# comfy-creator/Comfy-Gen-Server

Measured on AMD Instinct MI355X. Metric: images/sec (whole node) + sec/image, SDXL 1024 20-step Euler-a at 1/2/4/8 MI355X, higher is better.
Workload: dtype bf16; 1 GPU; model=sdxl-base, global_batch=8, seq_len=16384, resolution=1024, sampler_steps=20, sampler=euler_ancestral, unet_batch_per_gpu=16, parallelism=dp1, pipelined=True

## Files before the change

### build_native.py

```python
#!/usr/bin/env python3
from __future__ import annotations

import concurrent.futures as cf
import glob
import json
import os
import subprocess
import sys
import sysconfig

ROOT = os.path.dirname(os.path.abspath(__file__))
PKG = os.path.join(ROOT, "comfy_gen_server_amd")
KDIR = os.path.join(PKG, "csrc", "kernels")
RDIR = os.path.join(PKG, "csrc", "runtime")
LIB = os.path.join(PKG, "lib")
BUILD = os.path.join(ROOT, "build", "native")
ROCM = os.environ.get("ROCM_PATH", "/opt/rocm")
HIPCC = os.path.join(ROCM, "bin", "hipcc")
ARCH = os.environ.get("CGS_OFFLOAD_ARCH", "gfx950")


def _run(cmd):
    r = subprocess.run(cmd, stdout=subprocess.PIPE, stderr=subprocess.STDOUT, text=True)
    if r.returncode != 0:
        raise RuntimeError("command failed:\n" + " ".join(cmd) + "\n" + r.stdout)
    return r.stdout


def _stale(src, obj, deps=()):
    if not os.path.exists(obj):
        return True
    t = os.path.getmtime(obj)
    return any(os.path.getmtime(p) > t for p in (src,) + tuple(deps))


SCRATCH_BUDGET = {"gemm_bf16_nt_v7_kernel": 128, "conv_nhwc_v7_kernel": 128, "attn_fwd_d64": 64}


def _resources(out):
    res, cur = {}, None
    for line in out.splitlines():
        if "remark:" not in line:
            continue
        txt = line.split("remark:", 1)[1].split("[-Rpass", 1)[0].strip()
        key, _, val = txt.partition(":")
        val = val.strip()
        if key == "Function Name":
            cur = val
            res[cur] = {}
        elif cur is not None and key in ("VGPRs", "AGPRs", "ScratchSize [bytes/lane]", "VGPRs Spill"):
            res[cur][{"VGPRs": "vgpr", "AGPRs": "agpr", "ScratchSize [bytes/lane]": "scratch",
                      "VGPRs Spill": "spill"}[key]] = int(val.split()[0])
    return res


def _check_resources(report):
    if not report:
        return
    path = os.path.join(BUILD, "kernel_resources.json")
    old = {}
    if os.path.exists(path):
        with open(path) as f:
            old = json.load(f)
    old.update(report)
    with open(path, "w") as f:
        json.dump(old, f, indent=1, sort_keys=True)
    bad = [(k, v.get("scratch", 0), lim) for k, v in report.items() for pat, lim in SCRATCH_BUDGET.items()
           if pat in k and v.get("scratch", 0) > lim]
    if bad:
# ... 92 lines not shown
```

### comfy_gen_server_amd/_native.py

```python
from __future__ import annotations

import ctypes
import glob
import os
import threading

_HERE = os.path.dirname(os.path.abspath(__file__))
LIB_DIR = os.path.join(_HERE, "lib")
_lock = threading.Lock()
_kernels = None
_kernels_err = None


def kernel_lib_path() -> str:
    return os.environ.get("CGS_KERNELS_SO") or os.path.join(LIB_DIR, "libcgs_kernels.so")


def load_kernels():
    global _kernels, _kernels_err
    if _kernels is not None or _kernels_err is not None:
        return _kernels
    with _lock:
        if _kernels is not None or _kernels_err is not None:
            return _kernels
# ... 54 lines not shown
    "cgs_euler_step": [_P, _P, _P, _L, _F, _F, _F, _P],
    "cgs_timestep_embedding": [_P, _P, _I, _I, _F, _I, _P],
    "cgs_silu": [_P, _P, _L, _I, _P],
    "cgs_act": [_P, _P, _L, _I, _F, _I, _P],
    "cgs_upsample_nearest2x_nhwc": [_P, _P, _I, _I, _I, _I, _I, _P],
    "cgs_dwconv_nhwc": [_P, _P, _P, _P, _I, _I, _I, _I, _I, _I, _I, _P],
    "cgs_dwconv_ln_stats_nhwc": [_P, _P, _P, _P, _P, _I, _I, _I, _I, _I, _I, _F, _I, _P],
    "cgs_conv2d_nhwc": [_P, _P, _P, _P, _P, _I, _I, _I, _I, _I, _I, _I, _I, _I, _I, _I, _P],
    "cgs_fused_bias_act": [_P, _P, _P, _L, _I, _L, _F, _F, _I, _P],
    "cgs_upfirdn2d": [_P, _P, _P, _I, _I, _I, _I, _I, _I, _I, _I, _I, _I, _I, _I, _I, _I, _P],
    "cgs_resize": [_P, _P, _I, _I, _I, _I, _I, _I, _I, _I, _P],
    "cgs_lanczos_u8_h": [_P, _L, _L, _L, _L, _P, _I, _I, _I, _I, _I, _P, _P, _I, _I, _I, _P],
    "cgs_lanczos_u8_v": [_P, _I, _L, _L, _L, _L, _P, _I, _I, _I, _I, _P, _P, _I, _P],
    "cgs_bislerp": [_P, _P, _I, _I, _I, _I, _L, _L, _L, _L, _I, _I, _P, _P, _P, _I, _I, _P],
    "cgs_vq_nearest": [_P, _P, _P, _P, _I, _I, _I, _I, _P],
    "cgs_grn_nhwc": [_P, _P, _P, _P, _P, _I, _I, _I, _I, _P],
    "cgs_grn_stats": [_P, _P, _I, _I, _I, _I, _I, _P],
    "cgs_splitk_ws_bytes": [_I, _I, _I],
    "cgs_gemm_bf16_splitk": [_P, _P, _P, _P, _P, _P, _P, _I, _I, _I, _L, _L, _L, _L, _I, _F, _I, _I, _P, _L, _P],
    "cgs_grn_stats_gns": [_P, _P, _I, _I, _I, _P],
    "cgs_grn_apply_gns": [_P, _P, _P, _P, _P, _P, _I, _I, _I, _P],
    "cgs_gemm_bf16_gelu_gns": [_P, _P, _P, _P, _P, _P, _I, _I, _I, _L, _L, _L, _I, _P, _I, _P],
    "cgs_grn_scale_weight": [_P, _P, _P, _I, _I, _I, _I, _P, _P],
    "cgs_h2d_upload": [_P, _P, _L, _L, _I, _P],
    "cgs_gemm_f32": [_P, _P, _P, _P, _P, _I, _I, _I, _L, _L, _L, _L, _I, _F, _I, _I, _L, _L, _L, _P],
    "cgs_conv_f32": [_P, _P, _P, _P, _P, _P, _I, _I, _I, _I, _I, _I, _I, _I, _I, _I, _I, _I, _I, _P],
    "cgs_groupnorm_f32_ws": [_I, _I, _I],
    "cgs_groupnorm_f32": [_P, _P, _I, _P, _P, _P, _P, _P, _I, _I, _I, _I, _F, _I, _P],
    "cgs_layernorm_f32": [_P, _P, _P, _P, _L, _I, _F, _P],
    "cgs_softmax_rows": [_P, _P, _L, _I, _F, _I, _P],
    "cgs_gemm_bf16_w8": [_P, _P, _P, _P, _P, _I, _I, _I, _L, _L, _L, _L, _I, _F, _P],
    "cgs_gemm_bf16_v": [_P, _P, _P, _P, _P, _I, _I, _I, _L, _L, _L, _L, _I, _F, _I, _P],
    "cgs_conv2d_nhwc_v": [_P, _P, _I, _P, _P, _P, _P, _I, _I, _I, _I, _I, _I, _I, _I, _I, _I, _I, _I, _I, _P],
    "cgs_upconv_taps_nhwc": [_P, _P, _P, _P, _I, _I, _I, _I, _I, _P],
    "cgs_conv2d_nhwc_act": [_P, _P, _I, _P, _P, _P, _P, _I, _I, _I, _I, _I, _I, _I, _I, _I, _I, _I, _I, _I, _I, _F,
                            _P],
    "cgs_philox_randn": [_P, _I, _L, ctypes.c_ulonglong, _L, ctypes.c_ulonglong, _P, _F, _I, _P, _P],
    "cgs_euler_ancestral_philox": [_P, _P, _I, _L, _F, _F, _F, ctypes.c_ulonglong, _L, ctypes.c_ulonglong, _P, _P],
    "cgs_brownian_increment": [_P, _I, _L, ctypes.c_ulonglong, _L, ctypes.c_double, ctypes.c_double,
                               ctypes.c_double, ctypes.c_double, ctypes.c_double, _I, _F, _P, _P],
    "cgs_sampler_step_dev": [_P, _P, _P, _P, _I, _L, _F, _P, _I, _P, _P],
    "cgs_step_param": [_P, _I, _P, _I, _I, _P, _P],
    "cgs_step_advance": [_P, _P],
    "cgs_vae_out_u8": [_P, _P, _L, _P],
    "cgs_conv2d_nhwc_ex": [_P, _P, _I, _P, _P, _P, _P, _I, _I, _I, _I, _I, _I, _I, _I, _I, _I, _I, _I, _P],
    "cgs_region_accumulate": [_P, _P, _P, _I, _P, _I, _I, _I, _I, _I, _I, _I, _I, _I, _L, _L, _L, _L, _I, _L, _L,
                              _L, _L, _I, _F, _P],
    "cgs_region_normalize": [_P, _P, _P, _L, _I, _P],
    "cgs_clip_embed": [_P, _P, _P, _P, _I, _I, _I, _I, _I, _P],
    "cgs_pooled_gather": [_P, _P, _P, _I, _I, _I, _I, _P],
    "cgs_layernorm_stats": [_P, _P, _I, _I, _F, _I, _P],
    "cgs_gemm_bf16_lnfold": [_P, _P, _P, _P, _P, _P, _I, _I, _I, _L, _L, _L, _I, _P, _L, _P],
    "cgs_gemm_bf16_lnfold_v": [_P, _P, _P, _P, _P, _P, _I, _I, _I, _L, _L, _L, _I, _P, _L, _I, _P],
    "cgs_v7_ws_bytes": [_I, _I, _I],
    "cgs_v7_set_dbg": [_I],
    "cgs_v6_set_mode": [_I],
    "cgs_attn_set_prio": [_I],
    "cgs_gn_set_blocks": [_I],
    "cgs_conv_smalln_set_lds": [_I],
    "cgs_attn_set_kv2_rows": [_I],
    "cgs_grn_set_rows": [_I],
    "cgs_flash_attn_fwd_ks": [_P, _P, _P, _P, _I, _I, _I, _I, _L, _L, _L, _L, _L, _L, _L, _L, _F, _I, _P, _P, _P],
    "cgs_flash_attn_fwd_kv2": [_P, _P, _P, _P, _P, _P, _I, _I, _I, _I, _I, _L, _L, _L, _L, _L, _L, _L, _L, _L, _L, _L, _L, _F, _P],
    "cgs_conv2d_nhwc_gns": [_P, _P, _I, _P, _P, _P, _P, _I, _I, _I, _I, _I, _I, _I, _I, _I, _I, _I, _I, _P, _P],
    "cgs_groupnorm_band_stats": [_P, _P, _I, _P, _P, _P, _I, _I, _I, _I, _I, _P],
    "cgs_groupnorm_apply_stats": [_P, _P, _I, _P, _P, _P, _P, _P, _P, _I, _I, _I, _I, _I, _I, _P],
# ... 75 lines not shown
```

### comfy_gen_server_amd/csrc/kernels/conv.hip

```cpp
#include "common.h"
#include <stdlib.h>
#include "mfma_core.h"
#include "mfma_pp.h"
#include "mfma_pp160.h"
#include "mfma_ppk.h"

#define EPI_BIAS 1
#define EPI_RESIDUAL 2
#define CONV_UP2X 16
#ifndef CGS_CONV_PFE
#define CGS_CONV_PFE 0
#endif

typedef __attribute__((address_space(3))) void lds_void;

__device__ __attribute__((aligned(16))) unsigned char g_conv_zero_page[256];

struct ConvArgs {
  const u16* in;
  const u16* in2;
  const u16* w;
  const u16* bias;
  const u16* res;
  u16* out;
  int N, H, W, Cin, C1, Cout, kh, kw, stride, pad, Ho, Wo;
  int flags;
  int tiles_n;
  int group_m;
  unsigned cq_magic;
  int kw_m16;
  ppk::Split sp;
  float* gnp;
  int img_rsrc;
  int act;
  float act_param;
};

__device__ __forceinline__ mc::Epi conv_epi(const ConvArgs& a) {
  return mc::Epi{a.out, a.bias, a.res, a.Cout, a.Cout, a.flags & (EPI_BIAS | EPI_RESIDUAL), 1.0f};
}
__device__ __forceinline__ mc::Epi conv_tile_epi(const ConvArgs& a) {
  mc::Epi e = conv_epi(a);
  if (a.act) {
    e.flags |= MC_EPI_GELU;
    e.act = a.act;
    e.act_param = a.act_param;
  }
  return e;
}

static void conv_magic(ConvArgs& a) {
  const unsigned cq = (unsigned)(a.Cin / 64);
  a.cq_magic = cq <= 1 ? 0u : (unsigned)(((1ull << 32) + cq - 1) / cq);
  a.kw_m16 = (65536 + a.kw - 1) / a.kw;
}

static long long conv_tiles(ConvArgs& a, int BM, int BN) {
  const int M = a.N * a.Ho * a.Wo;
  a.tiles_n = (a.Cout + BN - 1) / BN;
  return (long long)((M + BM - 1) / BM) * a.tiles_n;
}

template <auto Kern>
static void conv_run(const ConvArgs& a, long long grid, int threads, int lds, hipStream_t stream) {
  max_dynamic_lds_once<Kern>(lds);
  Kern<<<(unsigned)grid, threads, lds, stream>>>(a);
}

// ... 311 lines not shown
    const bool ok = row < M;
    row = ok ? row : M - 1;
    const int hw = a->Ho * a->Wo;
    const int n = row / hw;
    const int rem = row - n * hw;
    const int oy = rem / a->Wo;
    const int py = oy * a->stride - a->pad, px = (rem - oy * a->Wo) * a->stride - a->pad;
    pix[s] = (n * a->H + py) * a->W + px;
    uint32_t m = 0;
    if (ok) {
      for (int ky = 0; ky < a->kh; ++ky) {
        const bool ry = (unsigned)(py + ky) < (unsigned)a->H;
        for (int kx = 0; kx < a->kw; ++kx)
          if (ry && (unsigned)(px + kx) < (unsigned)a->W) m |= 1u << (ky * a->kw + kx);
      }
    }
    vm[s] = m;
  }
  __device__ __forceinline__ void dma(int s, int k0, unsigned char* dst) const {
    const unsigned kq = (unsigned)k0 >> 6;
    const unsigned tap = a->cq_magic ? __umulhi(kq, a->cq_magic) : kq;
    const int ci0 = k0 - (int)tap * a->Cin;
    const int ky = (int)((tap * (unsigned)a->kw_m16) >> 16);
    const int kx = (int)tap - ky * a->kw;
    const bool second = ci0 >= a->C1;
    const int cs = second ? a->Cin - a->C1 : a->C1;
    const int cb = (second ? ci0 - a->C1 : ci0) + 8 * pp::src_chunk8(s & 1);
    const unsigned p = (unsigned)(pix[s] + ky * a->W + kx);
    const unsigned off = ((vm[s] >> tap) & 1u) ? 2u * (p * (unsigned)cs + (unsigned)cb) : 0x80000000u;
    __builtin_amdgcn_raw_ptr_buffer_load_lds(second ? r2 : r1, (lds_void*)dst, 16, off, 0, 0, 0);
  }
};

struct ConvGatherKD {
  static constexpr bool kOwnDMA = true;
  const ConvArgs* a;
  uint32_t pb1[4], pb2[4], vm[4];
  __amdgpu_buffer_rsrc_t r1, r2;
  __device__ __forceinline__ void make(long long n_img, unsigned px) {
    const unsigned c2 = (unsigned)(a->in2 ? a->Cin - a->C1 : a->C1);
    r1 = __builtin_amdgcn_make_buffer_rsrc((void*)(a->in + n_img * px * a->C1), 0, (int)(px * (unsigned)a->C1 * 2u),
                                           0x00020000);
    r2 = __builtin_amdgcn_make_buffer_rsrc((void*)((a->in2 ? a->in2 : a->in) + n_img * px * c2), 0,
                                           (int)(px * c2 * 2u), 0x00020000);
  }
  __device__ __forceinline__ void init() {
    if (!a->img_rsrc) make(0, (unsigned)(a->N * a->H * a->W));
  }
  __device__ __forceinline__ void tile(int m0) {
    if (a->img_rsrc) make(m0 / (a->Ho * a->Wo), (unsigned)(a->H * a->W));
  }
  __device__ __forceinline__ void setup(int s, int row) {
    const int M = a->N * a->Ho * a->Wo;
    const bool ok = row < M;
    row = ok ? row : M - 1;
    const int hw = a->Ho * a->Wo;
    const int n = row / hw;
    const int rem = row - n * hw;
    const int oy = rem / a->Wo;
    const int py = oy * a->stride - a->pad, px = (rem - oy * a->Wo) * a->stride - a->pad;
    const unsigned pix = (unsigned)(((a->img_rsrc ? 0 : n) * a->H + py) * a->W + px);
    uint32_t m = 0;
    if (ok) {
      for (int ky = 0; ky < a->kh; ++ky) {
        const bool ry = (unsigned)(py + ky) < (unsigned)a->H;
        for (int kx = 0; kx < a->kw; ++kx)
          if (ry && (unsigned)(px + kx) < (unsigned)a->W) m |= 1u << (ky * a->kw + kx);
      }
    }
    vm[s] = m;
    const unsigned ch = 16u * (unsigned)pp::src_chunk8(s & 1);
    pb1[s] = pix * (2u * (unsigned)a->C1) + ch;
    pb2[s] = pix * (2u * (unsigned)(a->Cin - a->C1)) + ch;
  }
  __device__ __forceinline__ void dma(int s, int k0, unsigned char* dst) const {
    const unsigned kq = (unsigned)k0 >> 6;
    const unsigned tap = __umulhi(kq, a->cq_magic) + (a->cq_magic ? 0u : kq);
    const int ci0 = k0 - (int)tap * a->Cin;
    const int ky = (int)((tap * (unsigned)a->kw_m16) >> 16);
    const int kx = (int)tap - ky * a->kw;
    const bool second = ci0 >= a->C1;
    const unsigned cs2 = 2u * (unsigned)(second ? a->Cin - a->C1 : a->C1);
    const unsigned so = (unsigned)(ky * a->W + kx) * cs2 + 2u * (unsigned)(second ? ci0 - a->C1 : ci0);
    const unsigned off = ((second ? pb2[s] : pb1[s]) + so) | (~(vm[s] << (31u - tap)) & 0x80000000u);
    __builtin_amdgcn_raw_ptr_buffer_load_lds(second ? r2 : r1, (lds_void*)dst, 16, off, 0, 0, 0);
  }
};

struct ConvGatherKU {
  static constexpr bool kOwnDMA = true;
  const ConvArgs* a;
  uint32_t pb[4], vm[4];
  int py[4], px[4];
  __amdgpu_buffer_rsrc_t r1;
  __device__ __forceinline__ void make(long long n_img, unsigned pixels) {
    r1 = __builtin_amdgcn_make_buffer_rsrc((void*)(a->in + n_img * pixels * a->C1), 0,
                                           (int)(pixels * (unsigned)a->C1 * 2u), 0x00020000);
  }
  __device__ __forceinline__ void init() {
    if (!a->img_rsrc) make(0, (unsigned)(a->N * a->H * a->W));
  }
  __device__ __forceinline__ void tile(int m0) {
    if (a->img_rsrc) make(m0 / (a->Ho * a->Wo), (unsigned)(a->H * a->W));
  }
  __device__ __forceinline__ void setup(int s, int row) {
    const int M = a->N * a->Ho * a->Wo;
    const bool ok = row < M;
    row = ok ? row : M - 1;
    const int hw = a->Ho * a->Wo;
    const int n = row / hw;
    const int rem = row - n * hw;
    const int oy = rem / a->Wo;
    const int y0 = oy * a->stride - a->pad, x0 = (rem - oy * a->Wo) * a->stride - a->pad;
    uint32_t m = 0;
    if (ok) {
      for (int ky = 0; ky < a->kh; ++ky) {
        const bool ry = (unsigned)(y0 + ky) < (unsigned)(2 * a->H);
        for (int kx = 0; kx < a->kw; ++kx)
          if (ry && (unsigned)(x0 + kx) < (unsigned)(2 * a->W)) m |= 1u << (ky * a->kw + kx);
      }
// ... 120 lines not shown
  const long long nwg = conv_tiles(a, pp::BM, pp::BN);
  const int kd = conv_kd(a);
  a.img_rsrc = kd == 2;
  if (!conv_fast_ok(a)) {
    const bool ku = (a.flags & CONV_UP2X) && g_conv_v6_ld != 0 && kd;
    if (ku) conv_magic(a);
    if (!ku) conv_run<conv_nhwc_v5_kernel<false>>(a, nwg, pp::THREADS, pp::LDS, stream);
    else conv_run<conv_nhwc_v5_kernel<true>>(a, nwg, pp::THREADS, pp::LDS, stream);
    return;
  }
  conv_magic(a);
  if (g_conv_v6_ld != 1 && kd) conv_run<conv_nhwc_v5k_kernel<true>>(a, nwg, pp::THREADS, pp::LDS, stream);
  else conv_run<conv_nhwc_v5k_kernel<false>>(a, nwg, pp::THREADS, pp::LDS, stream);
}

static int conv_pq_loader(ConvArgs& a) {
  const int kd = conv_kd(a);
  int ld = conv_fast_ok(a) ? (kd ? 2 : 1) : ((a.flags & CONV_UP2X) && kd ? 3 : 0);
  if (g_conv_v6_ld >= 0 && g_conv_v6_ld < ld) ld = ld == 3 ? 0 : g_conv_v6_ld;
  a.img_rsrc = ld >= 2 && kd == 2;
  if (ld) conv_magic(a);
  return ld;
}
template <typename F>
static void with_loader(int ld, F f) {
  if (ld == 3) f(std::integral_constant<int, 3>{});
  else if (ld == 2) f(std::integral_constant<int, 2>{});
  else if (ld == 1) f(std::integral_constant<int, 1>{});
  else f(std::integral_constant<int, 0>{});
}

template <int LD>
using ConvLoaderFor = typename std::conditional<
    LD == 3, ConvGatherKU,
    typename std::conditional<LD == 2, ConvGatherKD,
                              typename std::conditional<LD == 1, ConvGatherK<true>, ConvGatherA8>::type>::type>::type;
template <int LD, int DS = 0, bool GNS = false, int NJ = 5, int PFE = CGS_CONV_PFE>
__global__ __launch_bounds__(512) __attribute__((amdgpu_waves_per_eu(2, 2))) void conv_nhwc_v6_kernel(ConvArgs a) {
  extern __shared__ __attribute__((aligned(16))) unsigned char smem[];
  const int M = a.N * a.Ho * a.Wo;
  const int K = a.kh * a.kw * a.Cin;
  ConvLoaderFor<LD> al;
  al.a = &a;
  if constexpr (LD >= 2) al.init();
  mc::Epi e = conv_epi(a);
  e.gnp = a.gnp;
  e.hw = a.Ho * a.Wo;
  pq::run<decltype(al), false, DS, GNS, false, false, false, PFE, NJ>(al, a.w, K, M, a.Cout, K, e, smem,
                                                                              (M + pq::BM - 1) / pq::BM, a.tiles_n,
                                                                              a.group_m);
}

template <int LD>
__global__ __launch_bounds__(256) __attribute__((amdgpu_waves_per_eu(2, 2))) void conv_nhwc_v6w4_kernel(ConvArgs a) {
  extern __shared__ __attribute__((aligned(16))) unsigned char smem[];
  const int M = a.N * a.Ho * a.Wo;
  const int K = a.kh * a.kw * a.Cin;
  ConvLoaderFor<LD> al;
  al.a = &a;
  if constexpr (LD >= 2) al.init();
  mc::Epi e = conv_epi(a);
  using Gm = pq::Geo<5, 2, 4>;
  pq::run<decltype(al), false, 51, false, false, false, false, 0, 5, 2, 4>(al, a.w, K, M, a.Cout, K, e, smem,
                                                                          (M + Gm::BM - 1) / Gm::BM, a.tiles_n,
                                                                          a.group_m);
}

int v6_conv_ds();

template <int LD, int DS, bool GNS = false, int NJ = 5, int PFE = CGS_CONV_PFE>
static void conv_v6_launch(ConvArgs& a, int grid, hipStream_t stream) {
  conv_run<conv_nhwc_v6_kernel<LD, DS, GNS, NJ, PFE>>(a, grid, pq::THREADS, pq::Geo<NJ>::LDS, stream);
}

// ... 335 lines not shown
}

CGS_EXPORT int cgs_conv2d_nhwc_act(const void* x, const void* x2, int C1, const void* w, const void* bias,
                                   const void* res, void* out, int N, int H, int W, int Cin, int Cout, int kh, int kw,
                                   int stride, int pad, int Ho, int Wo, int flags, int variant, int act,
                                   float act_param, hipStream_t stream) {
  ConvArgs a = conv_args(x, x2, C1, w, bias, res, out, N, H, W, Cin, Cout, kh, kw, stride, pad, Ho, Wo, flags);
  if (!conv_shape_ok(a) || Cout <= 16 || Cout % 8 || (variant != 3 && variant != 4 && variant != 8) ||
      act < CGS_ACT_NONE || act > CGS_ACT_LEAKY_RELU)
    return (int)hipErrorInvalidValue;
  a.act = act;
  a.act_param = act_param;
  return conv_launch(a, stream, variant);
}

CGS_EXPORT int cgs_conv2d_nhwc_gns(const void* x, const void* x2, int C1, const void* w, const void* bias,
                                   const void* res, void* out, int N, int H, int W, int Cin, int Cout, int kh, int kw,
                                   int stride, int pad, int Ho, int Wo, int flags, float* gnp, hipStream_t stream) {
  ConvArgs a = conv_args(x, x2, C1, w, bias, res, out, N, H, W, Cin, Cout, kh, kw, stride, pad, Ho, Wo, flags);
  if (!gnp || ((uintptr_t)gnp % 16) || (Ho * Wo) % 256 || Cout % 8 || !conv_variant_ok(a, 6))
    return (int)hipErrorInvalidValue;
  a.gnp = gnp;
  conv_v6_go(a, stream);
  return (int)hipGetLastError();
}

CGS_EXPORT int cgs_conv2d_nhwc_v7ws(const void* x, const void* x2, int C1, const void* w, const void* bias,
                                    const void* res, void* out, int N, int H, int W, int Cin, int Cout, int kh, int kw,
                                    int stride, int pad, int Ho, int Wo, int flags, void* ws, long long ws_bytes,
                                    hipStream_t stream) {
  ConvArgs a = conv_args(x, x2, C1, w, bias, res, out, N, H, W, Cin, Cout, kh, kw, stride, pad, Ho, Wo, flags);
  return conv_shape_ok(a) ? conv_launch(a, stream, 7, ws, ws_bytes) : (int)hipErrorInvalidValue;
}
```

### comfy_gen_server_amd/models/layers.py

```python
from __future__ import annotations

import math

import torch
import torch.nn as nn

from .. import ops


class DerivedMixin:
    def _derived_get(self, key, fn):
        d = self.__dict__.setdefault("_derived", {})
        v = d.get(key)
        if v is None:
            v = fn()
            d[key] = v
        return v

    def invalidate_derived(self):
        self.__dict__["_derived"] = {}


WEIGHTS_EPOCH = 0

# ... 71 lines not shown
        if _hooked(self):
            return cast_bias_weight(self, x)
        w, b = self.weight, self.bias
        if w.dtype != x.dtype or w.device != x.device:
            w = w.to(device=x.device, dtype=x.dtype)
            b = None if b is None else b.to(device=x.device, dtype=x.dtype)
        return w, b


class Conv2d(nn.Module, DerivedMixin, CastWeightBiasOp):
    def __init__(self, in_channels, out_channels, kernel_size, stride=1, padding=0, bias=True,
                 groups=1, dtype=None, device=None, padding_mode="zeros"):
        super().__init__()
        if isinstance(kernel_size, int):
            kernel_size = (kernel_size, kernel_size)
        self.in_channels = in_channels
        self.out_channels = out_channels
        self.kernel_size = kernel_size
        self.stride = stride
        self.padding = padding
        self.groups = groups
        self.weight = nn.Parameter(torch.empty((out_channels, in_channels // groups) + tuple(kernel_size),
                                               dtype=dtype, device=device), requires_grad=False)
        if bias:
            self.bias = nn.Parameter(torch.empty(out_channels, dtype=dtype, device=device), requires_grad=False)
        else:
            self.register_parameter("bias", None)

    def weight_nhwc(self):
        return self._derived_get("w_nhwc", lambda: self.weight.permute(0, 2, 3, 1).contiguous())

    def weight_taps(self):
        return self._derived_get("w_taps", lambda: ops.core.upconv_tap_weights(self.weight))

    def forward(self, x, residual=None, upsample2x=False, x2=None, gn_stats=False, act=None, act_param=0.0):
        if _hooked(self):
            if x2 is not None:
                x = torch.cat([x, x2], dim=1)
            w, b = cast_bias_weight(self, x)
            return ops.conv2d(x, w, b, self.stride, self.padding, residual=residual, groups=self.groups,
                              upsample2x=upsample2x, act=act, act_param=act_param)
        w, b = self.weight, self.bias
        wn = None
        if x2 is not None:
            if x.is_cuda and self.groups == 1 and w.dtype == x.dtype and w.device == x.device:
                return ops.conv2d(x, w, b, self.stride, self.padding, residual=residual,
                                  weight_nhwc=self.weight_nhwc(), groups=self.groups, x2=x2, gn_stats=gn_stats,
                                  act=act, act_param=act_param)
            x = torch.cat([x, x2], dim=1)
        if w.dtype != x.dtype or w.device != x.device:
            w = w.to(device=x.device, dtype=x.dtype)
            b = None if b is None else b.to(device=x.device, dtype=x.dtype)
        elif x.is_cuda and self.groups == 1 and self.in_channels % 32 and x.dtype == torch.bfloat16 \
                and residual is None and not upsample2x:
            q = 32 if self.out_channels % 8 == 0 else 64
            cp = (self.in_channels + q - 1) // q * q
            pad = cp - self.in_channels
            w = self._derived_get("w_pad", lambda: torch.nn.functional.pad(self.weight, (0, 0, 0, 0, 0, pad)))
            wn = self._derived_get("w_nhwc_pad", lambda: w.permute(0, 2, 3, 1).contiguous())
            xp = torch.empty((x.shape[0], cp, x.shape[2], x.shape[3]), device=x.device, dtype=x.dtype,
                             memory_format=torch.channels_last)
            xp[:, self.in_channels:].zero_()
            xp[:, :self.in_channels] = x
            x = xp
        elif x.is_cuda and self.groups == 1:
            wn = self.weight_nhwc()
# ... 147 lines not shown
```

### comfy_gen_server_amd/models/unet.py

```python
from __future__ import annotations

import logging
import os

import torch
import torch.nn as nn

from .. import ops
from .attention import BasicTransformerBlock, SpatialTransformer, _Seq
from .layers import Conv2d, Conv3d, DerivedMixin, GroupNorm, Linear, _hooked, module_epoch


def _SKIPCAT():
    import os
    return os.environ.get("CGS_SKIPCAT", "1") != "0"


class SkipCat:
    __slots__ = ("a", "b")

    def __init__(self, a, b):
        self.a, self.b = a, b

    @property
# ... 1 lines not shown
        return torch.Size((self.a.shape[0], self.a.shape[1] + self.b.shape[1]) + tuple(self.a.shape[2:]))

    def materialize(self):
        h = torch.cat([self.a, self.b], dim=1)
        return h.contiguous(memory_format=torch.channels_last) if h.is_cuda else h


class ResBlock(nn.Module):
    def __init__(self, channels, emb_channels, out_channels=None, dtype=None, device=None,
                 kernel_size=3, skip_t_emb=False):
        super().__init__()
        out_channels = out_channels or channels
        self.channels = channels
        self.out_channels = out_channels
        self.skip_t_emb = skip_t_emb
        pad = kernel_size // 2
        self.in_layers = _Seq(GroupNorm(32, channels, dtype=dtype, device=device), nn.SiLU(),
                              Conv2d(channels, out_channels, kernel_size, padding=pad, dtype=dtype, device=device))
        if not skip_t_emb:
            self.emb_layers = _Seq(nn.SiLU(), Linear(emb_channels, out_channels, dtype=dtype, device=device))
        self.out_layers = _Seq(GroupNorm(32, out_channels, dtype=dtype, device=device), nn.SiLU(), nn.Dropout(0.0),
                               Conv2d(out_channels, out_channels, kernel_size, padding=pad, dtype=dtype, device=device))
        if out_channels == channels:
            self.skip_connection = nn.Identity()
        else:
            self.skip_connection = Conv2d(channels, out_channels, 1, dtype=dtype, device=device)

    def forward(self, x, emb_silu, transformer_options=None):
        if isinstance(x, SkipCat):
            if isinstance(self.skip_connection, nn.Identity):
                x = x.materialize()
            else:
                h = self.in_layers[2](self.in_layers[0](x.a, silu=True, x2=x.b), gn_stats=True)
                return self._out(h, emb_silu, self.skip_connection(x.a, x2=x.b))
        h = self.in_layers[0](x, silu=True)
        h = self.in_layers[2](h, gn_stats=True)
        skip = x if isinstance(self.skip_connection, nn.Identity) else None
        return self._out(h, emb_silu, skip if skip is not None else self.skip_connection(x))

    def _out(self, h, emb_silu, skip):
        pre = None
        if not self.skip_t_emb and emb_silu is not None:
            pj, off = getattr(emb_silu, "_cgs_emb_proj", None), self.__dict__.get("_cgs_emb_off")
            if pj is not None and off is not None:
                pre = pj[:, off:off + self.out_channels]
            else:
                pre = self.emb_layers[1](emb_silu).to(h.dtype)
        h = ops.group_norm(h, 32, self.out_layers[0].weight, self.out_layers[0].bias,
                           self.out_layers[0].eps, silu=True, pre_add=pre)
        return self.out_layers[3](h, residual=skip)


class Downsample(nn.Module):
    def __init__(self, channels, out_channels=None, dtype=None, device=None):
        super().__init__()
        self.op = Conv2d(channels, out_channels or channels, 3, stride=2, padding=1, dtype=dtype, device=device)

    def forward(self, x, *a, **k):
        return self.op(x)


class Upsample(nn.Module):
    def __init__(self, channels, out_channels=None, dtype=None, device=None):
        super().__init__()
        self.conv = Conv2d(channels, out_channels or channels, 3, padding=1, dtype=dtype, device=device)

    def forward(self, x, *a, output_shape=None, **k):
        if output_shape is not None and (output_shape[2] != 2 * x.shape[2] or output_shape[3] != 2 * x.shape[3]):
            x = torch.nn.functional.interpolate(x, size=output_shape[2:], mode="nearest")
        else:
            return self.conv(x, upsample2x=True)
        return self.conv(x)


class AlphaBlender(nn.Module):
    def __init__(self, alpha, merge_strategy="learned_with_images"):
        super().__init__()
        self.merge_strategy = merge_strategy
        if merge_strategy == "fixed":
            self.register_buffer("mix_factor", torch.tensor([float(alpha)]))
        elif merge_strategy in ("learned", "learned_with_images"):
            self.mix_factor = nn.Parameter(torch.tensor([float(alpha)]), requires_grad=False)
# ... 379 lines not shown
```

### comfy_gen_server_amd/models/vae.py

```python
from __future__ import annotations

import torch
import torch.nn as nn

from .. import ops
from .layers import Conv2d, Conv3d, GroupNorm, DerivedMixin


def _norm(c, dtype=None, device=None):
    return GroupNorm(32, c, eps=1e-6, dtype=dtype, device=device)


class ResnetBlock(nn.Module):
    def __init__(self, in_channels, out_channels=None, dtype=None, device=None, temb_channels=0):
        super().__init__()
        out_channels = out_channels or in_channels
        self.in_channels = in_channels
        self.out_channels = out_channels
        kw = dict(dtype=dtype, device=device)
        self.norm1 = _norm(in_channels, **kw)
        self.conv1 = Conv2d(in_channels, out_channels, 3, padding=1, **kw)
        self.norm2 = _norm(out_channels, **kw)
        self.conv2 = Conv2d(out_channels, out_channels, 3, padding=1, **kw)
        if in_channels != out_channels:
            self.nin_shortcut = Conv2d(in_channels, out_channels, 1, **kw)
        else:
            self.nin_shortcut = None

    def forward(self, x, temb=None):
        h = self.conv1(self.norm1(x, silu=True))
        h = self.norm2(h, silu=True)
        skip = x if self.nin_shortcut is None else self.nin_shortcut(x)
        return self.conv2(h, residual=skip)


class AttnBlock(nn.Module, DerivedMixin):
    def __init__(self, in_channels, dtype=None, device=None):
        super().__init__()
        kw = dict(dtype=dtype, device=device)
        self.in_channels = in_channels
        self.norm = _norm(in_channels, **kw)
        self.q = Conv2d(in_channels, in_channels, 1, **kw)
        self.k = Conv2d(in_channels, in_channels, 1, **kw)
        self.v = Conv2d(in_channels, in_channels, 1, **kw)
        self.proj_out = Conv2d(in_channels, in_channels, 1, **kw)

    def forward(self, x):
        b, c, h, w = x.shape
        hn = self.norm(x)
        tok = hn.permute(0, 2, 3, 1).reshape(b, h * w, c)
        if x.is_cuda and x.dtype == self.q.weight.dtype:
            wqkv = self._derived_get("w_qkv", lambda: torch.cat(
                [self.q.weight, self.k.weight, self.v.weight], 0).reshape(3 * c, c).contiguous())
            bqkv = self._derived_get("b_qkv", lambda: torch.cat([self.q.bias, self.k.bias, self.v.bias], 0))
            qkv = ops.linear(tok, wqkv, bqkv)
            q, k, v = qkv[..., :c], qkv[..., c:2 * c], qkv[..., 2 * c:]
            o = ops.attention(q, k, v, 1)
            res = x.permute(0, 2, 3, 1).reshape(b, h * w, c)
            wo = self._derived_get("w_o", lambda: self.proj_out.weight.reshape(c, c).contiguous())
            out = ops.linear(o, wo, self.proj_out.bias, residual=res if res.is_contiguous() else None)
            out = out.reshape(b, h, w, c).permute(0, 3, 1, 2)
            return out if res.is_contiguous() else out + x
        q = self.q(hn).permute(0, 2, 3, 1).reshape(b, h * w, c)
        k = self.k(hn).permute(0, 2, 3, 1).reshape(b, h * w, c)
        v = self.v(hn).permute(0, 2, 3, 1).reshape(b, h * w, c)
        o = ops.attention(q, k, v, 1)
# ... 186 lines not shown
```

### comfy_gen_server_amd/ops/__init__.py

```python
from . import dispatch
from .dispatch import (
    backend_for, set_backend_override, native_required, NativeMissingError, stats, reset_stats, torch_reference,
)
from .core import (
    linear, linear_geglu, attention, attention_lse, attention_kv2, attention_bias, group_norm, layer_norm, conv2d,
    conv_transpose2d, conv_transpose_phase_weights, silu, gelu, activation, ACT_CODES,
    upsample_nearest2x, timestep_embedding, cfg_combine, euler_step, depthwise_conv2d_nhwc,
    depthwise_conv2d_nhwc_lnstats,
    interpolate, fused_bias_act, channel_affine_nhwc, channel_affine_layernorm_nhwc, upfirdn2d, upfirdn2d_reference, vq_nearest, grn_nhwc,
    grn_fold_weight, softmax_rows,
    attention_with_probs, philox_randn, euler_ancestral_philox, brownian_increment, step_param, sampler_step_dev,
    step_advance, vae_out_u8, region_accumulate, region_normalize, clip_embed, pooled_gather,
    layernorm_stats, layernorm_stats_for, lnfold_weights, linear_lnfold, lnfold_available, fourier_filter, tome_match,
    rng_key_scope, lanczos_resize, lanczos_reference, lanczos_tables, bislerp, bislerp_tables,
)
```

### comfy_gen_server_amd/ops/core.py

```python
from __future__ import annotations

import collections
import math
import os

import numpy as np
import torch
import torch.nn.functional as F

from .. import _native
from . import autotune
from . import f32 as _f32
from .dispatch import backend_for, count, vendor_fallback

_DT = {torch.float32: 0, torch.bfloat16: 1, torch.float16: 2}

EPI_BIAS = 1
EPI_RESIDUAL = 2
EPI_GEGLU = 4
EPI_SILU_IN = 8
EPI_LNFOLD = 8
EPI_GELU = 32

_LIB_GEMM = os.environ.get("CGS_GEMM_LIB", "0") == "1"
# ... 928 lines not shown
                _check(_lib().cgs_upconv_taps_nhwc(xc.data_ptr(), wt.data_ptr(), _ptr(bias), out.data_ptr(), N, H, W,
                                                   Cin, Cout, _stream()), "cgs_upconv_taps_nhwc")
                return out

            if _upconv_use_taps(N, H, W, Cin, Cout, weight_taps is not None):
                return run_taps()
        if (gn_stats and variant == 6 and _GNS and (Ho * Wo) % 256 == 0 and Cin % 64 == 0 and C1 % 64 == 0
                and Cout % 8 == 0 and kh * kw * Cin >= 128 and (bias is None or bias.data_ptr() % 8 == 0)
                and _native.has_kernel("cgs_conv2d_nhwc_gns")):
            out = torch.empty((N, Cout, Ho, Wo), device=x.device, dtype=x.dtype, memory_format=torch.channels_last)
            part = torch.empty(N * (Ho * Wo // 64) * Cout * 2, device=x.device, dtype=torch.float32)
            _check(_lib().cgs_conv2d_nhwc_gns(*_conv_operands(xc, x2c, weight_nhwc, bias, r, out, kh, kw, stride,
                                                              padding, flags), part.data_ptr(), _stream()),
                   "cgs_conv2d_nhwc_gns")
            out._cgs_gnpart = (part, out.data_ptr())
            return out
        return run(variant)
    if upsample2x:
        x = upsample_nearest2x(x)
    if be == "torch":
        count("conv", "torch")
        y = F.conv2d(x.float(), weight.float(), None if bias is None else bias.float(), stride, padding,
                     groups=groups)
        if residual is not None:
            y = y + residual.float()
        return y.to(x.dtype)
    vendor_fallback("conv", f"dtype {x.dtype}, groups={groups}, Cin={x.shape[1]}, Cout={Cout}")
    y = F.conv2d(x, weight, bias, stride, padding, groups=groups)
    if residual is not None:
        y = y + residual
    return y


_CT_TAPS = ((3, 1), (2, 0))


def conv_transpose_phase_weights(weight: torch.Tensor):
    out = []
    for py in range(2):
        for px in range(2):
            wp = weight[:, :, list(_CT_TAPS[py])][:, :, :, list(_CT_TAPS[px])].permute(1, 0, 2, 3).contiguous()
            out.append((wp, wp.permute(0, 2, 3, 1).contiguous()))
    return out


def conv_transpose2d(x: torch.Tensor, weight: torch.Tensor, bias: torch.Tensor | None, stride=1, padding=0,
                     phase_weights=None) -> torch.Tensor:
    s = stride[0] if isinstance(stride, (tuple, list)) else stride
    p = padding[0] if isinstance(padding, (tuple, list)) else padding
    Cin, Cout, kh, kw = weight.shape
    be = backend_for("conv", x, "cgs_conv2d_nhwc")
    if (be == "hip" and x.dim() == 4 and x.dtype == torch.bfloat16 and weight.dtype == x.dtype and kh == kw == 4
            and s == 2 and p == 1 and Cin % 32 == 0 and (Cout % 8 == 0 or Cout <= 16)):
        N, _, H, W = x.shape
        pw = phase_weights if phase_weights is not None else conv_transpose_phase_weights(weight)
        out = torch.empty((N, Cout, 2 * H, 2 * W), device=x.device, dtype=x.dtype, memory_format=torch.channels_last)
        for i, (wp, wn) in enumerate(pw):
            py, px = divmod(i, 2)
            y = conv2d(x, wp, bias, 1, 1, weight_nhwc=wn)
            out[:, :, py::2, px::2] = y[:, :, py:py + H, px:px + W]
        return out
    if be == "torch":
        count("conv", "torch")
        y = F.conv_transpose2d(x.float(), weight.float(), None if bias is None else bias.float(), s, p)
        return y.to(x.dtype)
    vendor_fallback("conv", f"conv_transpose2d k={kh}x{kw} s={s} p={p} dtype {x.dtype}")
# ... 1043 lines not shown
```

Baseline: 3.479 images/s.

## Fuse 1x1 shortcut conv into residual-block output conv via K-tail gather

Adds a conv kernel variant that appends the 1x1 skip-connection conv as an extra K tail of the 3x3 output conv's implicit GEMM. The loader gathers from the shortcut input tensors once k passes the main K, and the weights and biases are concatenated. This removes the separate shortcut conv launch and the write and read of its intermediate residual tensor in UNet and VAE resblocks that have channel-changing skips. It is enabled only for a whitelist of shapes at sufficient batch size and falls back to the split path otherwise. The extra per-load select logic in the gather may cost registers.

```diff
diff --git a/build_native.py b/build_native.py
--- a/build_native.py
+++ b/build_native.py
@@ -34,7 +34,8 @@
     return any(os.path.getmtime(p) > t for p in (src,) + tuple(deps))
 
 
-SCRATCH_BUDGET = {"gemm_bf16_nt_v7_kernel": 128, "conv_nhwc_v7_kernel": 128, "attn_fwd_d64": 64}
+SCRATCH_BUDGET = {"gemm_bf16_nt_v7_kernel": 128, "conv_nhwc_v7_kernel": 128, "attn_fwd_d64": 64,
+                  "conv_nhwc_v6_kernel": 0}
 
 
 def _resources(out):
diff --git a/comfy_gen_server_amd/_native.py b/comfy_gen_server_amd/_native.py
--- a/comfy_gen_server_amd/_native.py
+++ b/comfy_gen_server_amd/_native.py
@@ -110,6 +110,7 @@
     "cgs_gemm_bf16_w8": [_P, _P, _P, _P, _P, _I, _I, _I, _L, _L, _L, _L, _I, _F, _P],
     "cgs_gemm_bf16_v": [_P, _P, _P, _P, _P, _I, _I, _I, _L, _L, _L, _L, _I, _F, _I, _P],
     "cgs_conv2d_nhwc_v": [_P, _P, _I, _P, _P, _P, _P, _I, _I, _I, _I, _I, _I, _I, _I, _I, _I, _I, _I, _I, _P],
+    "cgs_conv2d_nhwc_tail": [_P, _P, _I, _P, _P, _I, _I, _P, _P, _P, _I, _I, _I, _I, _I, _I, _I, _I, _I, _I, _P],
     "cgs_upconv_taps_nhwc": [_P, _P, _P, _P, _I, _I, _I, _I, _I, _P],
     "cgs_conv2d_nhwc_act": [_P, _P, _I, _P, _P, _P, _P, _I, _I, _I, _I, _I, _I, _I, _I, _I, _I, _I, _I, _I, _I, _F,
                             _P],
diff --git a/comfy_gen_server_amd/csrc/kernels/conv.hip b/comfy_gen_server_amd/csrc/kernels/conv.hip
--- a/comfy_gen_server_amd/csrc/kernels/conv.hip
+++ b/comfy_gen_server_amd/csrc/kernels/conv.hip
@@ -34,6 +34,10 @@
   int img_rsrc;
   int act;
   float act_param;
+  const u16* in3;
+  const u16* in4;
+  int C3, Ct;
+  int Km;
 };
 
 __device__ __forceinline__ mc::Epi conv_epi(const ConvArgs& a) {
@@ -411,17 +415,28 @@
   }
 };
 
-struct ConvGatherKD {
+template <bool TAIL>
+struct ConvGatherKDT {
   static constexpr bool kOwnDMA = true;
+  template <class T>
+  static __device__ __forceinline__ T pick(bool c, T x, T y) { return c ? x : y; }
   const ConvArgs* a;
   uint32_t pb1[4], pb2[4], vm[4];
-  __amdgpu_buffer_rsrc_t r1, r2;
+  uint32_t pb3[TAIL ? 4 : 1], pb4[TAIL ? 4 : 1];
+  __amdgpu_buffer_rsrc_t r1, r2, r3, r4;
   __device__ __forceinline__ void make(long long n_img, unsigned px) {
     const unsigned c2 = (unsigned)(a->in2 ? a->Cin - a->C1 : a->C1);
     r1 = __builtin_amdgcn_make_buffer_rsrc((void*)(a->in + n_img * px * a->C1), 0, (int)(px * (unsigned)a->C1 * 2u),
                                            0x00020000);
     r2 = __builtin_amdgcn_make_buffer_rsrc((void*)((a->in2 ? a->in2 : a->in) + n_img * px * c2), 0,
                                            (int)(px * c2 * 2u), 0x00020000);
+    if constexpr (TAIL) {
+      const unsigned c4 = (unsigned)(a->in4 ? a->Ct - a->C3 : a->C3);
+      r3 = __builtin_amdgcn_make_buffer_rsrc((void*)(a->in3 + n_img * px * a->C3), 0,
+                                             (int)(px * (unsigned)a->C3 * 2u), 0x00020000);
+      r4 = __builtin_amdgcn_make_buffer_rsrc((void*)((a->in4 ? a->in4 : a->in3) + n_img * px * c4), 0,
+                                             (int)(px * c4 * 2u), 0x00020000);
+    }
   }
   __device__ __forceinline__ void init() {
     if (!a->img_rsrc) make(0, (unsigned)(a->N * a->H * a->W));
@@ -451,6 +466,11 @@
     const unsigned ch = 16u * (unsigned)pp::src_chunk8(s & 1);
     pb1[s] = pix * (2u * (unsigned)a->C1) + ch;
     pb2[s] = pix * (2u * (unsigned)(a->Cin - a->C1)) + ch;
+    if constexpr (TAIL) {
+      const unsigned cp = (unsigned)(((a->img_rsrc ? 0 : n) * a->H + oy) * a->W + (rem - oy * a->Wo));
+      pb3[s] = cp * (2u * (unsigned)a->C3) + ch;
+      pb4[s] = cp * (2u * (unsigned)(a->Ct - a->C3)) + ch;
+    }
   }
   __device__ __forceinline__ void dma(int s, int k0, unsigned char* dst) const {
     const unsigned kq = (unsigned)k0 >> 6;
@@ -461,10 +481,21 @@
     const bool second = ci0 >= a->C1;
     const unsigned cs2 = 2u * (unsigned)(second ? a->Cin - a->C1 : a->C1);
     const unsigned so = (unsigned)(ky * a->W + kx) * cs2 + 2u * (unsigned)(second ? ci0 - a->C1 : ci0);
-    const unsigned off = ((second ? pb2[s] : pb1[s]) + so) | (~(vm[s] << (31u - tap)) & 0x80000000u);
-    __builtin_amdgcn_raw_ptr_buffer_load_lds(second ? r2 : r1, (lds_void*)dst, 16, off, 0, 0, 0);
+    if constexpr (!TAIL) {
+      const unsigned off = ((second ? pb2[s] : pb1[s]) + so) | (~(vm[s] << (31u - tap)) & 0x80000000u);
+      __builtin_amdgcn_raw_ptr_buffer_load_lds(second ? r2 : r1, (lds_void*)dst, 16, off, 0, 0, 0);
+    } else {
+      const unsigned moff = ((second ? pb2[s] : pb1[s]) + so) | (~(vm[s] << ((31u - tap) & 31u)) & 0x80000000u);
+      const bool tl = k0 >= a->Km;
+      const int ct = k0 - a->Km;
+      const bool t4 = ct >= a->C3;
+      const unsigned toff = pick(t4, pb4[s], pb3[s]) + 2u * (unsigned)(t4 ? ct - a->C3 : ct);
+      const __amdgpu_buffer_rsrc_t rm = pick(second, r2, r1), rt = pick(t4, r4, r3);
+      __builtin_amdgcn_raw_ptr_buffer_load_lds(pick(tl, rt, rm), (lds_void*)dst, 16, pick(tl, toff, moff), 0, 0, 0);
+    }
   }
 };
+using ConvGatherKD = ConvGatherKDT<false>;
 
 struct ConvGatherKU {
   static constexpr bool kOwnDMA = true;
@@ -651,14 +682,15 @@
 
 template <int LD>
 using ConvLoaderFor = typename std::conditional<
-    LD == 3, ConvGatherKU,
+    LD == 4, ConvGatherKDT<true>,
+    typename std::conditional<LD == 3, ConvGatherKU,
     typename std::conditional<LD == 2, ConvGatherKD,
-                              typename std::conditional<LD == 1, ConvGatherK<true>, ConvGatherA8>::type>::type>::type;
+                              typename std::conditional<LD == 1, ConvGatherK<true>, ConvGatherA8>::type>::type>::type>::type;
 template <int LD, int DS = 0, bool GNS = false, int NJ = 5, int PFE = CGS_CONV_PFE>
 __global__ __launch_bounds__(512) __attribute__((amdgpu_waves_per_eu(2, 2))) void conv_nhwc_v6_kernel(ConvArgs a) {
   extern __shared__ __attribute__((aligned(16))) unsigned char smem[];
   const int M = a.N * a.Ho * a.Wo;
-  const int K = a.kh * a.kw * a.Cin;
+  const int K = a.kh * a.kw * a.Cin + (LD == 4 ? a.Ct : 0);
   ConvLoaderFor<LD> al;
   al.a = &a;
   if constexpr (LD >= 2) al.init();
@@ -1060,3 +1092,31 @@
   ConvArgs a = conv_args(x, x2, C1, w, bias, res, out, N, H, W, Cin, Cout, kh, kw, stride, pad, Ho, Wo, flags);
   return conv_shape_ok(a) ? conv_launch(a, stream, 7, ws, ws_bytes) : (int)hipErrorInvalidValue;
 }
+
+#define CONV_TAIL_IMG 32
+CGS_EXPORT int cgs_conv2d_nhwc_tail(const void* x, const void* x2, int C1, const void* x3, const void* x4, int C3,
+                                    int Ct, const void* w, const void* bias, void* out, int N, int H, int W, int Cin,
+                                    int Cout, int kh, int kw, int pad, int flags, int variant, hipStream_t stream) {
+  ConvArgs a = conv_args(x, x2, C1, w, bias, nullptr, out, N, H, W, Cin, Cout, kh, kw, 1, pad, H, W, 0);
+  if ((variant != 6 && variant != 18) || !x3 || Ct < 64 || Ct % 64 || C3 < 64 || C3 % 64 ||
+      (x4 ? C3 >= Ct : C3 != Ct) || kh != 2 * pad + 1 || kw != 2 * pad + 1 || Cout % 8 || N < 1 || H < 1 || W < 1 ||
+      (long long)N * H * W >= (1ll << 31) || !conv_shape_ok(a) || !conv_fast_ok(a) || !conv_variant_ok(a, variant))
+    return (int)hipErrorInvalidValue;
+  a.in3 = (const u16*)x3;
+  a.in4 = (const u16*)x4;
+  a.C3 = C3;
+  a.Ct = Ct;
+  a.Km = kh * kw * Cin;
+  const int cmax = std::max(std::max(a.C1, Cin - a.C1), std::max(C3, Ct - C3));
+  const bool whole = (long long)N * H * W * cmax * 2 < (1ll << 31);
+  const bool img_ok = ((long long)H * W) % 256 == 0 && (long long)H * W * cmax * 2 < (1ll << 31);
+  if ((flags & CONV_TAIL_IMG) ? !img_ok : !(whole || img_ok)) return (int)hipErrorInvalidValue;
+  a.img_rsrc = (flags & CONV_TAIL_IMG) || !whole;
+  conv_magic(a);
+  const bool n128 = variant == 18;
+  const long long T = conv_tiles(a, pq::BM, n128 ? pq::Geo<4>::BN : pq::BN);
+  const int grid = (int)(T < num_cus() ? T : num_cus());
+  if (n128) conv_v6_launch<4, 51, false, 4, 0>(a, grid, stream);
+  else conv_v6_launch<4, 51>(a, grid, stream);
+  return (int)hipGetLastError();
+}
diff --git a/comfy_gen_server_amd/models/layers.py b/comfy_gen_server_amd/models/layers.py
--- a/comfy_gen_server_amd/models/layers.py
+++ b/comfy_gen_server_amd/models/layers.py
@@ -127,6 +127,25 @@
 
     def weight_taps(self):
         return self._derived_get("w_taps", lambda: ops.core.upconv_tap_weights(self.weight))
+
+    def weight_tail(self, shortcut: "Conv2d"):
+        tok = shortcut._derived_get("tail_tok", object)
+        v = self.__dict__.get("_derived", {}).get("w_tail")
+        if v is None or v[0] is not tok:
+            v = (tok,) + ops.core.conv_tail_weights(self.weight, self.bias, shortcut.weight, shortcut.bias)
+            self.__dict__.setdefault("_derived", {})["w_tail"] = v
+        return v[1], v[2]
+
+    def forward_tail(self, x, shortcut: "Conv2d", x3, x4=None):
+        w, ws = self.weight, shortcut.weight
+        if (_hooked(self) or _hooked(shortcut) or not x.is_cuda or self.groups != 1 or shortcut.groups != 1
+                or self.stride != 1 or shortcut.stride != 1 or shortcut.padding != 0
+                or tuple(shortcut.kernel_size) != (1, 1) or w.dtype != x.dtype or w.device != x.device
+                or ws.dtype != x.dtype or ws.device != x.device or self.in_channels % 32):
+            return self(x, residual=shortcut(x3, x2=x4))
+        return ops.conv2d_tail(x, w, self.bias, (x3, x4), ws, shortcut.bias, self.padding,
+                               weight_tail=lambda: self.weight_tail(shortcut),
+                               split=lambda: self(x, residual=shortcut(x3, x2=x4)))
 
     def forward(self, x, residual=None, upsample2x=False, x2=None, gn_stats=False, act=None, act_param=0.0):
         if _hooked(self):
diff --git a/comfy_gen_server_amd/models/unet.py b/comfy_gen_server_amd/models/unet.py
--- a/comfy_gen_server_amd/models/unet.py
+++ b/comfy_gen_server_amd/models/unet.py
@@ -57,13 +57,14 @@
                 x = x.materialize()
             else:
                 h = self.in_layers[2](self.in_layers[0](x.a, silu=True, x2=x.b), gn_stats=True)
-                return self._out(h, emb_silu, self.skip_connection(x.a, x2=x.b))
+                return self._out(h, emb_silu, None, (x.a, x.b))
         h = self.in_layers[0](x, silu=True)
         h = self.in_layers[2](h, gn_stats=True)
-        skip = x if isinstance(self.skip_connection, nn.Identity) else None
-        return self._out(h, emb_silu, skip if skip is not None else self.skip_connection(x))
-
-    def _out(self, h, emb_silu, skip):
+        if isinstance(self.skip_connection, nn.Identity):
+            return self._out(h, emb_silu, x)
+        return self._out(h, emb_silu, None, (x, None))
+
+    def _out(self, h, emb_silu, skip, sc_in=None):
         pre = None
         if not self.skip_t_emb and emb_silu is not None:
             pj, off = getattr(emb_silu, "_cgs_emb_proj", None), self.__dict__.get("_cgs_emb_off")
@@ -73,6 +74,8 @@
                 pre = self.emb_layers[1](emb_silu).to(h.dtype)
         h = ops.group_norm(h, 32, self.out_layers[0].weight, self.out_layers[0].bias,
                            self.out_layers[0].eps, silu=True, pre_add=pre)
+        if sc_in is not None:
+            return self.out_layers[3].forward_tail(h, self.skip_connection, sc_in[0], sc_in[1])
         return self.out_layers[3](h, residual=skip)
 
 
diff --git a/comfy_gen_server_amd/models/vae.py b/comfy_gen_server_amd/models/vae.py
--- a/comfy_gen_server_amd/models/vae.py
+++ b/comfy_gen_server_amd/models/vae.py
@@ -30,8 +30,9 @@
     def forward(self, x, temb=None):
         h = self.conv1(self.norm1(x, silu=True))
         h = self.norm2(h, silu=True)
-        skip = x if self.nin_shortcut is None else self.nin_shortcut(x)
-        return self.conv2(h, residual=skip)
+        if self.nin_shortcut is None:
+            return self.conv2(h, residual=x)
+        return self.conv2.forward_tail(h, self.nin_shortcut, x)
 
 
 class AttnBlock(nn.Module, DerivedMixin):
diff --git a/comfy_gen_server_amd/ops/__init__.py b/comfy_gen_server_amd/ops/__init__.py
--- a/comfy_gen_server_amd/ops/__init__.py
+++ b/comfy_gen_server_amd/ops/__init__.py
@@ -4,6 +4,7 @@
 )
 from .core import (
     linear, linear_geglu, attention, attention_lse, attention_kv2, attention_bias, group_norm, layer_norm, conv2d,
+    conv2d_tail, conv_tail_weights,
     conv_transpose2d, conv_transpose_phase_weights, silu, gelu, activation, ACT_CODES,
     upsample_nearest2x, timestep_embedding, cfg_combine, euler_step, depthwise_conv2d_nhwc,
     depthwise_conv2d_nhwc_lnstats,
diff --git a/comfy_gen_server_amd/ops/core.py b/comfy_gen_server_amd/ops/core.py
--- a/comfy_gen_server_amd/ops/core.py
+++ b/comfy_gen_server_amd/ops/core.py
@@ -984,6 +984,78 @@
     return y
 
 
+def conv_tail_weights(weight: torch.Tensor, bias, weight_sc: torch.Tensor, bias_sc):
+    Cout = weight.shape[0]
+    w = torch.cat([weight.permute(0, 2, 3, 1).reshape(Cout, -1), weight_sc.reshape(Cout, -1).to(weight.dtype)],
+                  1).contiguous()
+    if bias is None and bias_sc is None:
+        return w, None
+    b = sum(t.float() for t in (bias, bias_sc) if t is not None)
+    return w, b.to(weight.dtype)
+
+
+_CONV_TAIL_SHAPES = {(128, 128, 320, 960, 320): 16, (128, 128, 320, 640, 320): 16, (64, 64, 640, 320, 640): 16,
+                     (1024, 1024, 128, 256, 128): 8}
+
+
+def _conv_tail_variant(Cout: int) -> str:
+    return "v6n128" if Cout % 128 == 0 and Cout % 160 else "v6"
+
+
+def _conv_use_tail(N, H, W, Cin, Ct, Cout, cached) -> bool:
+    mode = os.environ.get("CGS_CONV_TAIL", "")
+    if mode in ("0", "1"):
+        return mode == "1"
+    return cached and N >= _CONV_TAIL_SHAPES.get((H, W, Cin, Ct, Cout), 1 << 30)
+
+
+def conv2d_tail(x: torch.Tensor, weight: torch.Tensor, bias, tail, weight_sc: torch.Tensor, bias_sc, padding=1,
+                weight_nhwc=None, weight_sc_nhwc=None, weight_tail=None, split=None) -> torch.Tensor:
+    x3, x4 = tail
+    pd = padding[0] if isinstance(padding, (tuple, list)) else padding
+
+    def _split():
+        skip = conv2d(x3, weight_sc, bias_sc, 1, 0, weight_nhwc=weight_sc_nhwc, x2=x4)
+        return conv2d(x, weight, bias, 1, pd, residual=skip, weight_nhwc=weight_nhwc)
+    if split is None:
+        split = _split
+
+    Cout, Cin, kh, kw = weight.shape
+    C3 = x3.shape[1]
+    Ct = C3 + (0 if x4 is None else x4.shape[1])
+    if not (_spatial() is None and x.dim() == 4 and backend_for("conv", x, "cgs_conv2d_nhwc") == "hip"
+            and x.dtype == torch.bfloat16 and weight.dtype == x.dtype and weight_sc.dtype == x.dtype
+            and x3.dtype == x.dtype and (x4 is None or x4.dtype == x.dtype)
+            and kh == kw == 2 * pd + 1 and tuple(weight_sc.shape) == (Cout, Ct, 1, 1) and x.shape[1] == Cin
+            and Cin % 64 == 0 and C3 % 64 == 0 and Ct % 64 == 0 and Cout % 8 == 0 and Cout > 16
+            and x3.shape[0] == x.shape[0] and x3.shape[2:] == x.shape[2:]
+            and (x4 is None or (x4.shape[0] == x.shape[0] and x4.shape[2:] == x.shape[2:]))
+            and _native.has_kernel("cgs_conv2d_nhwc_tail")):
+        return split()
+    N, _, H, W = x.shape
+    if not _conv_use_tail(N, H, W, Cin, Ct, Cout, weight_tail is not None):
+        return split()
+    choice = autotune.choose(("conv", N, H, W, Cin, Cout, kh, 1, pd, 0, 0, "tail", Ct)
+                             + ((("dual", C3),) if x4 is not None else ()), [(_conv_tail_variant(Cout), None)])
+    wt = weight_tail() if callable(weight_tail) else weight_tail
+    if wt is None:
+        wt = conv_tail_weights(weight, bias, weight_sc, bias_sc)
+    wf, bf = wt
+    if bf is not None and bf.data_ptr() % 8:
+        return split()
+    count("conv", "hip")
+    count("conv_tail", "hip")
+    xc = x.contiguous(memory_format=torch.channels_last)
+    x3c = x3.contiguous(memory_format=torch.channels_last)
+    x4c = None if x4 is None else x4.contiguous(memory_format=torch.channels_last)
+    out = torch.empty((N, Cout, H, W), device=x.device, dtype=x.dtype, memory_format=torch.channels_last)
+    flags = 32 if os.environ.get("CGS_CONV_TAIL_IMG", "") == "1" else 0
+    _check(_lib().cgs_conv2d_nhwc_tail(xc.data_ptr(), None, Cin, x3c.data_ptr(), _ptr(x4c), C3, Ct, wf.data_ptr(),
+                                       _ptr(bf), out.data_ptr(), N, H, W, Cin, Cout, kh, kw, pd, flags,
+                                       CONV_VARIANTS[choice], _stream()), "cgs_conv2d_nhwc_tail")
+    return out
+
+
 _CT_TAPS = ((3, 1), (2, 0))
 
 
```

Result: no change. 3.490 images/s, median of 6 (+0.3%).
